# brucefan1983/GPUMD

Measured on AMD Instinct MI355X. Metric: atom-steps/sec, NEP PbTe NVE (nep4 2 Te Pb, examples/nep_train/nep.txt), higher is better.
Workload: dtype f32

## Files before the change

### gpumd_amd/csrc/capi_impl.h

```cpp
#pragma once
#include "../../include/nepmi.h"
#include "engine_impl.h"

#include <exception>
#include <string>

struct nepmi_api;
#if defined(NEPMI_CAPI_DISPATCH)
extern "C" const nepmi_api nepmi_self_api;
#define NEPMI_SELF_API (&nepmi_self_api)
#else
#define NEPMI_SELF_API nullptr
#endif

struct nepmi_model {
  const nepmi_api* api;
  nepmi::NepModel m;
};

struct nepmi_engine {
  const nepmi_api* api;
  nepmi::EngineT<NepmiBackend>* e;
};

// ... 981 lines not shown
  const std::string n(name);
  const int iv = (int)value;
  auto& eng = *e->e;
  if (n == "generic")
    return guarded([&] { eng.set_force_generic(iv != 0); });
  if (n == "tiles")
    eng.set_tile_mode(iv < 0 ? -1 : iv > 2 ? 2 : iv);
  else if (n == "win_lanes")
    eng.set_win_lanes(iv);
  else if (n == "win_max_atoms")
    eng.set_win_max_atoms(iv);
  else if (n == "scatter_guard")
    eng.set_scatter_guard_delayed(value, eng.take_guard_delay());
  else if (n == "scatter_guard_hard")
    eng.set_scatter_guard(-1.0, value);
  else if (n == "scatter_guard_delay")
    eng.set_guard_delay(iv);
  else if (n == "radial_mask")
    eng.set_radial_mask(iv != 0);
  else if (n == "radial_sync")
    eng.set_radial_sync(iv != 0);
  else if (n == "angular_fused")
    eng.set_angular_fused(iv != 0);
  else if (n == "angular_pair_trip")
    eng.set_angular_pair_trip(iv != 0);
  else if (n == "angular_flat_tables")
    eng.set_angular_flat_tables(iv != 0);
  else if (n == "lean_list_walks")
    eng.set_lean_list_walks(iv != 0);
  else if (n == "angular_only_list_a")
    eng.set_angular_only_list_a(iv != 0);
  else if (n == "rebuild_fast_pack")
    eng.set_rebuild_fast_pack(iv != 0);
  else if (n == "fold_seam")
    eng.set_fold_seam(iv != 0);
  else if (n == "brick_force") {
    if (iv != 0 && !eng.has_brick_force())
      return fail(NEPMI_ERR_ARG, "option 'brick_force': the per-brick force kernel is not part of this build (make BRICK=1)");
    eng.set_brick_force(iv != 0);
  }
  else if (n == "win_static")
    eng.set_win2(iv != 0);
  else if (n == "keep_lists_on_box_change")
    eng.set_keep_lists(iv != 0);
  else if (n == "stepwise_loops")
    eng.set_stepwise_loops(iv != 0);
  else if (n == "mfma")
    eng.set_use_mfma(iv);
  else if (n == "angular_recompute")
    eng.set_angular_recompute(iv);
  else
    return fail(NEPMI_ERR_ARG, "unknown engine option '" + n + "'");
  return NEPMI_OK;
}

}
```

### gpumd_amd/csrc/engine.hip

```cpp
#include <hip/hip_runtime.h>
#include <hiprand/hiprand_kernel.h>

#include <cstring>
#include <stdexcept>
#include <string>

#include "engine_impl.h"
#include "nep_scatter.h"
#include "nep_fused.h"
#ifndef NEPMI_WITH_BRICK
#define NEPMI_WITH_BRICK 0
#endif
#if NEPMI_WITH_BRICK
#include "experimental/nep_brick.h"
#endif

namespace nepmi {

#define NEPMI_HIP_CHECK(expr)                                                                       \
  do {                                                                                              \
    hipError_t err__ = (expr);                                                                      \
    if (err__ != hipSuccess)                                                                        \
      throw std::runtime_error(std::string("HIP error: ") + hipGetErrorString(err__) + " at " +     \
                               __FILE__ + ":" + std::to_string(__LINE__) + " (" #expr ")");         \
// ... 325 lines not shown
  body.lds_stage(nepmi_lds_pairs_s, tid, BLOCK);
  if (tid < 64)
    hist[tid] = 0;
  const unsigned per_xcd = gridDim.x >> 3;
  const unsigned tile = (blockIdx.x & 7u) * per_xcd + (blockIdx.x >> 3);
  const int64_t base = (int64_t)tile * (BLOCK / 2);
  const int j = tid >> 1;
  const bool live = base + j < n;
  int key = 0;
  if (live) {
    key = body.sort_key(base + j);
    key = key > 63 ? 63 : key;
    if (tile & 1u)
      key = 63 - key;
  }
  __syncthreads();
  if (live && (tid & 1) == 0)
    atomicAdd(&hist[key], 1);
  __syncthreads();
  if (tid == 0) {
    int run = 0;
    for (int c = 63; c >= 0; --c) {
      const int h = hist[c];
      hist[c] = run;
      run += h;
    }
  }
  __syncthreads();
  if (live && (tid & 1) == 0)
    perm[atomicAdd(&hist[key], 1)] = (unsigned short)j;
  __syncthreads();
  if (live)
    body.template run_parts<2>(base + perm[j], tid & 1, (lds_cfloat_ptr)nepmi_lds_pairs_s);
}

template <class Body>
__global__ void __launch_bounds__(256) nepmi_fused_image(const Body body, float* img)
{
  body.lds_stage(img, (int)threadIdx.x, 256);
}

template <int BLOCK, int P, class Body>
__global__ void __launch_bounds__(BLOCK) nepmi_kernel_lds_parts(const Body body, const int64_t n, const int* frozen)
{
  extern __shared__ __attribute__((aligned(16))) float nepmi_lds_parts[];
  if (frozen && *frozen != 0)
    return;
  const unsigned per_xcd = gridDim.x >> 3;
  const unsigned tile = (blockIdx.x & 7u) * per_xcd + (blockIdx.x >> 3);
  const int64_t i = ((int64_t)tile * BLOCK + threadIdx.x) / P;
  if (i < n)
    body.template run_parts<P>(i, (int)(threadIdx.x % P), (lds_cfloat_ptr)nepmi_lds_parts);
}

template <int BLOCK>
__device__ __forceinline__ int block_exclusive_scan(int v, int* total);

template <class Body>
__global__ void __launch_bounds__(kWinThreads) __attribute__((amdgpu_waves_per_eu(Body::kMinWavesPerEu)))
nepmi_win_kernel(const Body body, const int64_t nbricks)
{
  extern __shared__ __attribute__((aligned(16))) char nepmi_win_lds[];
  NEPMI_LDS(char)* lds = (NEPMI_LDS(char)*)nepmi_win_lds;
  if (body.skip())
    return;
  const unsigned per_xcd = gridDim.x >> 3;
// ... 1109 lines not shown
    const bool t = timed(slot);
    if (t)
      timer_start(timing->slot[slot]);
    hipLaunchKernelGGL((nepmi_kernel_lds_parts<BLOCK, P, Body>), dim3((unsigned)grid), dim3(BLOCK), lds_bytes, stream, body, n,
                       frozen);
    NEPMI_HIP_CHECK(hipGetLastError());
    if (t)
      timer_stop(timing->slot[slot]);
  }

  template <int BLOCK, class Body, bool SORTED = false>
  void launch_lds_pairs(int slot, int64_t n, const Body& body)
  {
    if (n <= 0)
      return;
    const int64_t grid = ((2 * n + BLOCK - 1) / BLOCK + 7) / 8 * 8;
    const size_t lds_bytes = ((size_t)body.lds_floats() * sizeof(float) + 15) / 16 * 16;
    void (*kern)(const Body, const int64_t, const int*) = nullptr;
    if constexpr (SORTED)
      kern = &nepmi_kernel_lds_pairs_sorted<BLOCK, Body>;
    else
      kern = &nepmi_kernel_lds_pairs<BLOCK, Body>;
    if (lds_bytes > 60 * 1024)
      NEPMI_HIP_CHECK(hipFuncSetAttribute(reinterpret_cast<const void*>(kern), hipFuncAttributeMaxDynamicSharedMemorySize, (int)lds_bytes));
    const bool t = timed(slot);
    if (t)
      timer_start(timing->slot[slot]);
    hipLaunchKernelGGL(kern, dim3((unsigned)grid), dim3(BLOCK), lds_bytes, stream, body, n, frozen);
    NEPMI_HIP_CHECK(hipGetLastError());
    if (t)
      timer_stop(timing->slot[slot]);
  }

  template <class S>
  size_t fused_image_floats(const ModelD& md, bool flat = false) const
  {
    return (size_t)fused_lds_layout<S>(md, 0, flat ? 1 : 0).total;
  }
  template <class S>
  void launch_angular_fused(int slot, int64_t n, const ModelD& md, const Bufs& b, int export_qfp, float* img, bool build, bool pair_trip,
                            bool flat = false)
  {
    if (build) {
      if (flat)
        hipLaunchKernelGGL((nepmi_fused_image<AngularFusedBody<S, 0, 1>>), dim3(1), dim3(256), 0, stream,
                           AngularFusedBody<S, 0, 1>{md, b, export_qfp, nullptr}, img);
      else
        hipLaunchKernelGGL((nepmi_fused_image<AngularFusedBody<S>>), dim3(1), dim3(256), 0, stream,
                           AngularFusedBody<S>{md, b, export_qfp, nullptr}, img);
      NEPMI_HIP_CHECK(hipGetLastError());
    }
#ifndef NEPMI_AFU_BLOCK
#define NEPMI_AFU_BLOCK 256
#endif
#ifndef NEPMI_AFU_SORT
#define NEPMI_AFU_SORT 0
#endif
    constexpr bool kTrips = FusedShape<S>::NLOC <= kFusedTripMaxChannels;
    if (flat) {
      if constexpr (kTrips) {
        if (pair_trip) {
          launch_lds_pairs<NEPMI_AFU_BLOCK, AngularFusedBody<S, 1, 1>, NEPMI_AFU_SORT != 0>(slot, n, AngularFusedBody<S, 1, 1>{md, b, export_qfp, img});
          return;
        }
      }
      launch_lds_pairs<NEPMI_AFU_BLOCK, AngularFusedBody<S, 0, 1>, NEPMI_AFU_SORT != 0>(slot, n, AngularFusedBody<S, 0, 1>{md, b, export_qfp, img});
      return;
    }
    if constexpr (kTrips) {
      if (pair_trip) {
        launch_lds_pairs<NEPMI_AFU_BLOCK, AngularFusedBody<S, 1>, NEPMI_AFU_SORT != 0>(slot, n, AngularFusedBody<S, 1>{md, b, export_qfp, img});
        return;
      }
    }
    launch_lds_pairs<NEPMI_AFU_BLOCK, AngularFusedBody<S>, NEPMI_AFU_SORT != 0>(slot, n, AngularFusedBody<S>{md, b, export_qfp, img});
  }

  template <class S>
  size_t fused_window_lds_bytes(const ModelD& md) const
  {
    return (size_t)fused_lds_layout<S>(md, kFusedWindowTypes).total * sizeof(float);
  }
  static constexpr bool kHasFusedWindow = NEPMI_WITH_FUSED_WINDOW != 0;
  template <class S>
  void launch_angular_fused_window(int slot, int64_t n, const ModelD& md, const Bufs& b, int export_qfp, float* img, bool build)
  {
#if NEPMI_WITH_FUSED_WINDOW
    if (n <= 0)
      return;
    AngularFusedBody<S> body{md, b, export_qfp, nullptr};
    if (build) {
      hipLaunchKernelGGL((nepmi_fused_image<AngularFusedBody<S>>), dim3(1), dim3(256), 0, stream, body, img);
      NEPMI_HIP_CHECK(hipGetLastError());
    }
    body.img = img;
    body.tw = kFusedWindowTypes;
    const int64_t grid = ((n + 127) / 128 + 7) / 8 * 8;
    const size_t lds_bytes = (fused_window_lds_bytes<S>(md) + 15) / 16 * 16;
    if (lds_bytes > 64 * 1024)
      NEPMI_HIP_CHECK(hipFuncSetAttribute(reinterpret_cast<const void*>(&nepmi_fused_window_kernel<AngularFusedBody<S>>),
                                          hipFuncAttributeMaxDynamicSharedMemorySize, (int)lds_bytes));
    const bool t = timed(slot);
    if (t)
      timer_start(timing->slot[slot]);
    hipLaunchKernelGGL((nepmi_fused_window_kernel<AngularFusedBody<S>>), dim3((unsigned)grid), dim3(256), lds_bytes, stream, body, n, frozen);
    NEPMI_HIP_CHECK(hipGetLastError());
    if (t)
      timer_stop(timing->slot[slot]);
// ... 428 lines not shown
```

### gpumd_amd/csrc/engine_impl.h

```cpp
#pragma once
#include "nep_bodies.h"
#include "nep_md.h"
#include "nep_corr.h"
#include "nep_rdf.h"
#include "nep_adf.h"
#include "nep_orient.h"
#include "nep_model.h"
#include "nep_window.h"
#include "nep_highl.h"
#include "tersoff_bodies.h"

#include <cmath>
#include <cstdio>
#include <cstring>
#include <string>
#include <random>
#include <vector>

#ifndef NEPMI_TERSOFF_SEAM
#define NEPMI_TERSOFF_SEAM 1
#endif
#ifndef NEPMI_WIN2_DEFAULT
#define NEPMI_WIN2_DEFAULT 1
#endif
// ... 1514 lines not shown
          const int64_t nc = set_grid();
          be_.memset(b_.cell_count, 0, sizeof(int) * (nc + 1));
          be_.memset(b_.flags + kFlagMaxBrick, 0, sizeof(int));
          be_.template launch<256>(kSlotMisc, N_, BinAtomsBody{box_, b_, pos});
          be_.template launch<64>(kSlotMisc, nc / 64, BrickMaxBody{b_});
          int fullest = 0;
          be_.sync();
          be_.d2h(&fullest, b_.flags + kFlagMaxBrick, sizeof(int));
          if (fullest <= kBrickFill)
            best = rc_cell;
        }
        grid_edge_ = best;
        grid_n_ = N_;
        for (int k = 0; k < 9; ++k)
          grid_h_[k] = box_.h[k];
      }
      rc_cell = grid_edge_;
      bin_grid();
      ncell = set_grid();
    }
    set_metric(false);
    be_.memset(b_.cell_count, 0, sizeof(int) * (ncell + 1));
    be_.memset(b_.cell_fill, 0, sizeof(int) * ncell);
    be_.memset(b_.cell_ghost, 0, sizeof(int) * ncell);
    const bool fast = rebuild_fast_pack_;
    static_assert(kFlagMaxAng == kFlagMaxSkin + 1 && kFlagMaxWindow == kFlagMaxAng + 1 && kFlagMaxCell == kFlagMaxWindow + 2, "adjacent flag words");
    if (fast) {
      be_.memset(b_.flags + kFlagMaxSkin, 0, 5 * sizeof(int));
    } else {
      be_.memset(b_.flags + kFlagMaxSkin, 0, 2 * sizeof(int));
    }
    be_.memset(b_.flags + kFlagMoved, 0, sizeof(int));
    be_.memset(b_.flags + kFlagOutlier, 0, sizeof(int));
    be_.begin_region(kRegionRebuild);
    be_.template launch<256>(kSlotMisc, N_, BinAtomsBody{box_, b_, pos});
    be_.exclusive_scan(b_.cell_count, ncell + 1, scan_scratch_);
    be_.template launch<256>(kSlotMisc, N_, FillCellsBody{b_});
    be_.template launch<256>(kSlotMisc, ncell, SortCellsBody{b_});
    be_.template launch<256>(kSlotMisc, N_, GatherSortedBody{box_, b_, pos, type});
    if (fuse_ann_active()) {
      be_.template launch<256>(kSlotMisc, N_, IdentityOrderBody{b_});
    } else {
      const int64_t nkeys = ((N_ >> kTypeChunkShift) + 1) * model_.num_types;
      be_.memset(b_.tcount, 0, sizeof(int) * (nkeys + 1));
      be_.template launch<64>(kSlotMisc, nkeys, TypeCountBody{b_, model_.num_types});
      be_.exclusive_scan(b_.tcount, nkeys + 1, scan_scratch_);
      be_.template launch<256>(kSlotMisc, N_, TypeFillBody{b_, model_.num_types});
    }
    if (!fast)
      be_.memset(b_.flags + kFlagMaxWindow, 0, 3 * sizeof(int));
    num_bricks_ = (int64_t)b_.gbx * b_.gby * b_.gbz;
    b_.brick_live = (b_.level && brick_live_buf_) ? brick_live_buf_ : nullptr;
    if (b_.level) {
      be_.memset(brick_live_buf_, 0, sizeof(int) * (size_t)(num_bricks_ + 1));
      be_.template launch<256>(kSlotMisc, N_, MarkGhostCellsBody{b_});
    }
    bool wave_stats = false;
    if constexpr (B::kHasScatter) {
      if (fast) {
        be_.launch_tile_stats_wave(kSlotMisc, num_bricks_, box_, b_);
        wave_stats = true;
      }
    }
    if (!wave_stats)
      be_.template launch<64>(kSlotMisc, num_bricks_, TileStatsBody{box_, b_});
    be_.memset(b_.brick_flag + num_bricks_, 0, sizeof(int));
// ... 166 lines not shown
  }
  bool ang_fused_window_active() const
  {
    if (!B::kHasFusedWindow || !B::kHasFusedAngular || !ang_fused_ || model_.kind != 0 || shape_ == 0 || ann_mode_ != 1 || model_.num_types <= 4 || !b_.fpr)
      return false;
    if ((model_.n_max_angular + 2) / 2 > 5)
      return false;
    const int nrh = (model_.n_max_radial + 2) / 2, nloc = (model_.n_max_angular + 2) / 2;
    const int dph = (nrh + model_.num_L * nloc + 3) / 4 * 4;
    const size_t T = (size_t)model_.num_types, tw = 4;
    const size_t floats = tw * ((size_t)model_.num_neurons * 2 * dph + 32 + 2 * model_.num_neurons) + 2 * dph +
                          tw * T * ((model_.n_max_angular + 1) * (model_.basis_size_angular + 1) + 1) + 16;
    return floats * sizeof(float) <= 80 * 1024;
  }
  template <class S>
  void launch_angular_fused_window(int export_qfp = 0)
  {
    if constexpr (B::kHasFusedWindow && B::kHasFusedAngular && S::fixed && S::TS == 0) {
      const size_t need = be_.template fused_image_floats<S>(md_);
      if (!fused_img_ || fused_img_floats_ < need) {
        dfree(fused_img_);
        fused_img_ = dalloc<float>(need);
        fused_img_floats_ = need;
        fused_img_stale_ = true;
      }
      be_.template launch_angular_fused_window<S>(kSlotAngular, N_, md_, b_, export_qfp, fused_img_, fused_img_stale_);
      fused_img_stale_ = false;
    }
  }
  template <class S>
  void launch_angular_fused(int export_qfp = 0, bool classic_image = false)
  {
    if constexpr (B::kHasFusedAngular && S::fixed) {
      if (ang_flat_tables_ && !classic_image) {
        const size_t need = be_.template fused_image_floats<S>(md_, true);
        if (!fused_img_flat_ || fused_img_flat_floats_ < need) {
          dfree(fused_img_flat_);
          fused_img_flat_ = dalloc<float>(need);
          fused_img_flat_floats_ = need;
          fused_img_flat_stale_ = true;
        }
        be_.template launch_angular_fused<S>(kSlotAngular, N_, md_, b_, export_qfp, fused_img_flat_, fused_img_flat_stale_, ang_pair_trip_, true);
        fused_img_flat_stale_ = false;
        last_ang_flat_ = true;
        return;
      }
      const size_t need = be_.template fused_image_floats<S>(md_);
      if (!fused_img_ || fused_img_floats_ < need) {
        dfree(fused_img_);
        fused_img_ = dalloc<float>(need);
        fused_img_floats_ = need;
        fused_img_stale_ = true;
      }
      be_.template launch_angular_fused<S>(kSlotAngular, N_, md_, b_, export_qfp, fused_img_, fused_img_stale_, ang_pair_trip_);
      fused_img_stale_ = false;
      last_ang_flat_ = false;
    }
  }

  template <class S>
  bool brick_force_wanted(const WinStage& ws2) const
  {
    if constexpr (!(B::kHasBrickForce && S::fixed && S::TS == 2)) {
      return false;
    } else {
      if (!brick_force_ || !ang_fused_active() || b_.level || b_.use_rmask || b_.use_csync || !scatter_wanted<S>(ws2))
        return false;
      return be_.template brick_lds_bytes<S>(md_, win_.wmax) <= B::kMaxLdsBytes;
    }
  }
  template <class S>
  void launch_brick_force(const WinStage& ws2, const int* frozen)
  {
    if constexpr (B::kHasBrickForce && S::fixed && S::TS == 2) {
      if (fused_img_stale_ || !fused_img_) {
        launch_angular_fused<S>(0, true);
      }
      be_.template launch_brick_force<S>(kSlotAngular, kSlotForce, num_bricks_, N_, ws2, md_, halo_, fmap_, fold_rows_, step_outputs_,
                                         fused_img_, frozen);
    }
  }

  template <class S>
  void launch_angular_force()
  {
    const bool big_table = (size_t)cang_floats(md_) * sizeof(float) > 16 * 1024;
#ifndef NEPMI_AF_PAIRS_BIG
// ... 196 lines not shown
    temperature_ = temperature;
    const float qT = (float)temperature * m.q_scaler_temp;
    b0_eff_.resize(m.b0.size());
    for (size_t k = 0; k < m.b0.size(); ++k)
      b0_eff_[k] = m.b0[k] - m.w0_temp[k] * qT;
    be_.h2d(const_cast<float*>(md_.b0), b0_eff_.data(), sizeof(float) * b0_eff_.size());
    be_.ann_prepare(md_, b_);
    fused_img_stale_ = fused_img_flat_stale_ = true;
  }
  double temperature() const { return temperature_; }
  bool temperature_model() const { return model_.temperature_model; }
  int recompute_s() const
  {
    return recompute_mode_ < 0 ? (model_.MN_angular <= 16 ? 1 : 0) : (recompute_mode_ ? 1 : 0);
  }
  void adopt_from(const EngineT& o)
  {
    use_tiles_ = o.use_tiles_;
    tile_mode_ = o.tile_mode_;
    recompute_mode_ = o.recompute_mode_;
    win_lanes_ = o.win_lanes_;
    win_max_atoms_ = o.win_max_atoms_;
    use_win2_ = o.use_win2_;
    external_skin_ = o.external_skin_;
    force_form_ = o.force_form_;
    use_rmask_ = o.use_rmask_;
    use_csync_ = o.use_csync_;
    ang_fused_ = o.ang_fused_;
    ang_pair_trip_ = o.ang_pair_trip_;
    ang_flat_tables_ = o.ang_flat_tables_;
    lean_walks_ = o.lean_walks_;
    aonly_list_a_ = o.aonly_list_a_;
    rebuild_fast_pack_ = o.rebuild_fast_pack_;
    fold_seam_ = o.fold_seam_;
    brick_force_ = o.brick_force_;
    loop_ctx_ = o.loop_ctx_;
    scatter_disabled_ = o.scatter_disabled_;
    b_.scatter_limit = o.b_.scatter_limit;
    b_.fold_guard = o.b_.fold_guard;
    b_.scatter_hard = o.b_.scatter_hard;
    b_.fold_hard = o.b_.fold_hard;
    hard_factor_ = o.hard_factor_;
    hard_asked_ = o.hard_asked_;
    guard_delay_ = o.guard_delay_;
    guard_delayed_ = o.guard_delayed_;
    if (reverse_ghosts_ != o.reverse_ghosts_)
      set_reverse_ghosts(o.reverse_ghosts_);
    unwrapped_ = o.unwrapped_;
    nhc_fresh_ = o.nhc_fresh_;
    bdp_rng_ = o.bdp_rng_;
    bdp_iset_ = o.bdp_iset_;
    bdp_gset_ = o.bdp_gset_;
    lan_seed_ = o.lan_seed_;
    num_compute = o.num_compute;
    num_rebuild = o.num_rebuild;
    num_discarded = o.num_discarded;
    num_range_handovers = o.num_range_handovers;
    be_.adopt_options(o.be_);
    if (ann_mode_ != o.ann_mode_)
      set_use_mfma(o.ann_mode_);
    if (force_generic_ != o.force_generic_)
      set_force_generic(o.force_generic_);
    if (o.temperature_ != temperature_)
      set_temperature(o.temperature_);
    have_list_ = false;
  }
// ... 347 lines not shown
    b_.fold_hard = on ? (int)((hard_factor_ > 2.0 ? hard_factor_ : 2.0) * b_.scatter_limit * 4194304.0) : 0;
  }
  bool scatter_enabled() const { return !scatter_disabled_; }
  void clear_range_hard()
  {
    int ov = 0;
    be_.d2h(&ov, b_.flags + kFlagOverflow, sizeof(int));
    if (ov & kOverflowRangeHard) {
      ov &= ~kOverflowRangeHard;
      be_.h2d(b_.flags + kFlagOverflow, &ov, sizeof(int));
    }
  }
  void disable_scatter()
  {
    if (!scatter_disabled_)
      ++num_range_handovers;
    scatter_disabled_ = true;
    be_.memset(b_.flags + kFlagRange, 0, sizeof(int));
  }
  bool last_scatter_form() const { return last_scatter_form_; }
  void set_angular_fused(bool on) { ang_fused_ = on; }
  void set_angular_pair_trip(bool on) { ang_pair_trip_ = on; }
  bool ang_pair_trip_active() const { return ang_pair_trip_ && (model_.n_max_angular + 2) / 2 <= 4; }
  void set_angular_flat_tables(bool on) { ang_flat_tables_ = on; }
  void set_lean_list_walks(bool on) { lean_walks_ = on; }
  void set_angular_only_list_a(bool on)
  {
    if (on != aonly_list_a_)
      have_list_ = false;
    aonly_list_a_ = on;
  }
  bool aonly_list_a_active() const { return aonly_list_a_ && shape_ts() == 2 && !use_rmask_; }
  void set_rebuild_fast_pack(bool on) { rebuild_fast_pack_ = on; }
  template <class S>
  bool lean_radial() const
  {
    return lean_walks_ && S::TS > 0;
  }
  bool lean_scatter() const { return lean_walks_ && shape_ts() > 0; }
  void set_fold_seam(bool on) { fold_seam_ = on; }
  void set_brick_force(bool on) { brick_force_ = on; }
  static constexpr bool has_brick_force() { return B::kHasBrickForce; }
  void set_loop_context(bool on) { loop_ctx_ = on; }
  void set_step_outputs(bool on) { step_outputs_ = on; }
  bool loop_context() const { return loop_ctx_; }
  void exact_virials()
  {
    if (!virial_local_ || model_.kind != 0 || last_small_)
      return;
    be_.frozen = nullptr;
    NEPMI_SHAPE_DISPATCH(exact_virials_shape, 1, ())
  }
  bool virial_local() const { return virial_local_; }

private:
  template <class S>
  void compact_lists_shape()
  {
    const bool padded_rows = b_.use_csync != 0;
    force_kernels_shape<S>(kPhaseRadialOnly, nullptr);
    if (padded_rows)
      angular_kernels<S>();
  }
  template <class S>
  void exact_virials_shape()
  {
// ... 60 lines not shown
    std::string s;
    if (model_.kind == 1)
      return "potential=tersoff1989 kernels=bond_order+force(fp64)";
    if (shape_ == 6) {
      char jb[96];
      std::snprintf(jb, sizeof jb, "shape=jit(%d,%d,%d,%d,%d;%s)", model_.n_max_radial, model_.basis_size_radial, model_.n_max_angular,
                    model_.basis_size_angular, model_.num_L, model_.num_types <= 2 ? std::to_string(model_.num_types).c_str() : "T");
      s += jb;
    } else {
      if (shape_ == 7 || shape_ == 8 || shape_ == 9) {
        s += shape_ == 7 ? "shape=cover(8,12,8,12,6;T)" : (shape_ == 8 ? "shape=cover(12,16,10,12,6;T)" : "shape=cover(8,12,8,12,6;2)");
        if (model_.embedded()) {
          char eb[128];
          std::snprintf(eb, sizeof eb, "<-zero_padded_model(%d,%d,%d,%d,%d)", model_.file_n_max_radial, model_.file_basis_size_radial,
                        model_.file_n_max_angular, model_.file_basis_size_angular, model_.file_num_L);
          s += eb;
        }
      } else {
        s += std::string("shape=") + shapes[shape_ >= 0 && shape_ <= 5 ? shape_ : 0];
      }
    }
    if (last_small_)
      return s + " path=small_box(all image pairs)";
    const int lanes = win_lanes();
    const bool win2 = win2_ok_ && lanes == 1;
    s += tile_ok_ ? (win2 ? " window=lds_static" : " window=lds_scanned") : " window=none(gather kernels)";
    s += " lanes_per_atom=" + std::to_string(tile_ok_ ? lanes : 1);
    if (last_brick_)
      s += " force=one_kernel_per_brick(descriptor+ann+partial_forces+lds_scatter_of_own_halves,lane_pairs)";
    else if (last_ang_fused_ && last_ang_window_)
      s += " angular=descriptor+ann+partial_forces_in_one_kernel(lane_pairs,sums_in_registers,type_sorted,window_of_4_types)";
    else if (last_ang_fused_)
      s += std::string(" angular=descriptor+ann+partial_forces_in_one_kernel(lane_pairs,sums_in_registers") +
           (ang_pair_trip_active() ? ",two_record_trips" : "") + (last_ang_flat_ ? ",flat_tables)" : ")");
    else if (fuse_ann_active())
      s += " ann=fused_with_angular_descriptor(packed_fp32,no_mfma)";
    else if (ann_mode_ != 0 && b_.ann_img && (model_.num_types <= 4 || b_.skip_atab))
      s += model_.num_types > 4 ? " ann=mfma_f32_32x32x2(one_type_per_workgroup)" : " ann=mfma_f32_32x32x2";
    else
      s += " ann=per_atom";
    if (!last_ang_fused_) {
      s += (shape_ != 0 && model_.n_max_angular + 1 >= 7) ? " angular_force=lane_pairs" : " angular_force=one_lane";
      s += recompute_s() ? " angular_sums=recomputed" : " angular_sums=stored";
    }
    s += (tile_ok_ && win2 && shape_ts() > 0 && lean_walks_) ? " list_walks=lean" : " list_walks=classic";
    s += (tile_ok_ && win2 && aonly_built_) ? " list_a=angular_only" : " list_a=classic";
    s += rebuild_fast_pack_ ? (b_.tbits ? " rebuild=fast_pack(types_from_the_builder)" : " rebuild=fast_pack") : " rebuild=classic";
    s += (last_scatter_form_ && last_mask_form_)   ? " radial_list=inside_bits_over_the_verlet_words"
         : (last_scatter_form_ && last_sync_form_) ? " radial_list=wave_synchronous_words"
                                                   : " radial_list=compacted";
    s += last_scatter_form_ ? (last_fold_seam_ ? " force_assembly=lds_scatter_of_own_halves(fixed_point)+fold_in_integrator_pass"
                                               : " force_assembly=lds_scatter_of_own_halves(fixed_point)+fold") :
         last_rows_form_ ? " force_assembly=table_rows_in_lds"
                         : (last_fpj_form_ ? " force_assembly=neighbour_half_from_fp_rows" : " force_assembly=table_rows_gathered");
    if (num_seam_vetoes_ > 0)
      s += " seam_vetoes=" + std::to_string(num_seam_vetoes_);
    if (tile_ok_)
      s += " bricks=" + std::to_string(num_bricks_) + " window_slots=" + std::to_string(win_.wmax);
    return s;
  }
  void force_kernels(int phase, const int* frozen = nullptr)
  {
    be_.frozen = frozen;
    force_kernels_dispatch(phase, frozen);
    be_.frozen = nullptr;
    step_outputs_ = true;
    assembly_part_ = 0;
// ... 20 lines not shown
        be_.template launch_lds<kTersoffBlock>(kSlotRadial, N_, TersoffPartialBody{box_, tp_, b_, tb_});
      if (tersoff_defer_)
        tersoff_deferred_ = true;
      else
        be_.template launch<64>(kSlotForce, N_, TersoffAssembleBody{b_, tb_});
      be_.end_region(kRegionForce);
      return;
    }
    NEPMI_SHAPE_DISPATCH(force_kernels_shape, 1, (phase, frozen))
  }

  NepModel model_;
  B be_;
  int64_t cap_;
  int64_t N_;
  ModelD md_{};
  Bufs b_;
  BoxD box_;
  WinLayout win_{0, 0};
  bool win2_ok_ = false, use_win2_ = NEPMI_WIN2_DEFAULT != 0;
  bool use_rows_ = true;
  bool last_rows_form_ = false, last_fpj_form_ = false, last_scatter_form_ = false;
  int force_form_ = -1;
  bool loop_ctx_ = false;
  bool virial_local_ = false;
  double hard_factor_ = 4.0;
  bool ang_fused_ = true;
  bool ang_pair_trip_ = !(std::getenv("NEPMI_ANGULAR_PAIR_TRIP") && std::atoi(std::getenv("NEPMI_ANGULAR_PAIR_TRIP")) == 0);
  bool ang_flat_tables_ = !(std::getenv("NEPMI_ANGULAR_FLAT_TABLES") && std::atoi(std::getenv("NEPMI_ANGULAR_FLAT_TABLES")) == 0);
  bool lean_walks_ = !(std::getenv("NEPMI_LEAN_LIST_WALKS") && std::atoi(std::getenv("NEPMI_LEAN_LIST_WALKS")) == 0);
  bool aonly_list_a_ = !(std::getenv("NEPMI_ANGULAR_ONLY_LIST_A") && std::atoi(std::getenv("NEPMI_ANGULAR_ONLY_LIST_A")) == 0);
  bool aonly_built_ = false;
  bool rebuild_fast_pack_ = !(std::getenv("NEPMI_REBUILD_FAST_PACK") && std::atoi(std::getenv("NEPMI_REBUILD_FAST_PACK")) == 0);
  float* fused_img_flat_ = nullptr;
  size_t fused_img_flat_floats_ = 0;
  bool fused_img_flat_stale_ = true;
  bool last_ang_flat_ = false;
  bool brick_force_ = false;
  bool last_brick_ = false;
  bool brick_pending_ = false;
  float* fused_img_ = nullptr;
  size_t fused_img_floats_ = 0;
  bool fused_img_stale_ = true;
  bool last_ang_fused_ = false;
  bool use_rmask_ = false;
  bool last_mask_form_ = false;
  bool last_ang_window_ = false;
  bool last_sync_form_ = false;
  int guard_delay_ = 0;
  int guard_delay_next_ = 0;
  bool fold_seam_ = !(std::getenv("NEPMI_FOLD_SEAM") && std::atoi(std::getenv("NEPMI_FOLD_SEAM")) == 0);
  bool fold_defer_ = false;
  bool fold_deferred_ = false;
  static constexpr int kSeamBackoffSteps = 256;
  int seam_backoff_ = 0;
  int64_t num_seam_vetoes_ = 0;
  bool last_fold_seam_ = false;
  bool tersoff_defer_ = false;
  bool tersoff_deferred_ = false;
  int64_t calm_steps_ = 0;
  int* brick_live_buf_ = nullptr;
  double* thermo_rows_ = nullptr;
  int64_t thermo_rows_cap_ = 0;
  bool rev_valid_ = false;
  const int* dmap_dev_ = nullptr;
  double hard_asked_ = 4.0;
// ... 77 lines not shown
```

### gpumd_amd/csrc/nep_bodies.h

```cpp
#pragma once
#include <type_traits>

#include "nep_dev.h"

namespace nepmi {

struct alignas(16) F4 {
  float x, y, z;
  int w;
};

struct alignas(16) U4 {
  unsigned x, y, z, w;
};

struct alignas(16) WinRec {
  int x, y, z;
  int w;
};

struct WinGeom {
  double inv_unit;
  double cell_frac[3];
  int cv[9];
// ... 9 lines not shown
#define NEPMI_ATOMIC_MAX(ptr, v) atomicMax((ptr), (v))
#else
NEPMI_HD int host_fetch_add(int* p, int v) { int o = *p; *p = o + v; return o; }
#define NEPMI_ATOMIC_ADD(ptr, v) host_fetch_add((ptr), (v))
#define NEPMI_ATOMIC_OR(ptr, v) (*(ptr) |= (v))
#define NEPMI_ATOMIC_MAX(ptr, v) (*(ptr) = (*(ptr) > (v) ? *(ptr) : (v)))
#endif

template <int NR_, int KR_, int NA_, int KA_, int NL_, int TS_>
struct Shape {
  static constexpr int NR = NR_, KR = KR_, NA = NA_, KA = KA_, NL = NL_, TS = TS_;
  static constexpr bool fixed = NR_ >= 0;
  static constexpr int NRM = NR_ >= 0 ? NR_ : 19;
  static constexpr int KRM = KR_ >= 0 ? KR_ : 19;
  static constexpr int NAM = NA_ >= 0 ? NA_ : 19;
  static constexpr int KAM = KA_ >= 0 ? KA_ : 19;
  static constexpr int NLM = NL_ >= 0 ? NL_ : 14;
  static constexpr int kRows = NR_ >= 0 ? 6 : 14;
  static constexpr int DIMM = (NRM + 1) + (NAM + 1) * NLM;
};
using ShapeGeneric = Shape<-1, -1, -1, -1, -1, 0>;

enum FlagSlot {
  kFlagMoved = 0, kFlagOverflow = 1,
  kFlagRange = 2,
  kFlagMaxSkin = 3, kFlagMaxAng = 4,
  kFlagMaxWindow = 5, kFlagMaxBrick = 6, kFlagMaxCell = 7, kFlagNumBoundary = 8,
  kFlagOutlier = 9,
  kFlagFoldRows = 10,
  kFlagSeamVeto = 11,
  kNumFlags = 12
};
constexpr int kOverflowRangeHard = 16;

constexpr int kAngRowPad = 8;
constexpr int kNullRecord = -1;
struct Bufs {
  int64_t N;
  int nbx, nby, nbz;
  int gbx, gby, gbz;
  double rc_inv_cell;
  float rc_skin_sq;
  float rc_askin_sq;
  int* cell_count;
  int* cell_fill;
  int* cell_ghost;
  int* brick_live;
  int* brick_flag;
  int* brick_order;
  int* cid;
  int* perm;
  PosQ* posq;
  double* x0s;
  int MN_skin, MN_ang, MN_acomp;
  int MN_arows;
  int* nn_ang;   int* nl_ang;  unsigned short* rev_ang;
  int* nn_skin;  int* nl_skin;
  unsigned short* code_ang;
  unsigned short* code_skin;
  int* nn_rad;   F4* rstash;
  int* nn_angstep; F4* acomp;
  int* nn_angtrue;
  unsigned short* amap;
  F4* f12;
  float* q;
  float* fp;
// ... 2730 lines not shown
```

### gpumd_amd/nep.py

```python
import ctypes as C
import weakref

import numpy as np

from . import _capi


def _h9(box):
    h = np.ascontiguousarray(np.asarray(box, dtype=np.float64).reshape(9))
    return h, h.ctypes.data_as(_capi.c_dp)


def _pbc3(pbc):
    p = np.ascontiguousarray(np.asarray(pbc, dtype=np.int32).reshape(3))
    return p, p.ctypes.data_as(_capi.c_ip)


class Model:

    def __init__(self, path, lib=None):
        from . import load_library
        self.lib = lib if lib is not None else load_library()
        self.path = path
        self.handle = self.lib.nepmi_model_load(path.encode())
# ... 313 lines not shown
    def set_radial_mask(self, on=True):
        self.set_option("radial_mask", 1 if on else 0)

    def set_radial_sync(self, on=True):
        self.set_option("radial_sync", 1 if on else 0)

    def set_scatter_guard(self, ev_per_angstrom=64.0, hard_factor=0.0):
        self.set_option("scatter_guard", float(ev_per_angstrom))
        self.set_option("scatter_guard_hard", float(hard_factor))

    def set_virial_mode(self, mode=0):
        self._ck(self.lib.nepmi_engine_set_virial_mode(self.handle, int(mode)))

    def set_brick_force(self, on=True):
        self.set_option("brick_force", 1 if on else 0)

    def set_angular_fused(self, on=True):
        self.set_option("angular_fused", 1 if on else 0)

    def set_angular_pair_trip(self, on=True):
        self.set_option("angular_pair_trip", 1 if on else 0)

    def set_angular_flat_tables(self, on=True):
        self.set_option("angular_flat_tables", 1 if on else 0)

    def set_lean_list_walks(self, on=True):
        self.set_option("lean_list_walks", 1 if on else 0)

    def set_angular_only_list_a(self, on=True):
        self.set_option("angular_only_list_a", 1 if on else 0)

    def set_rebuild_fast_pack(self, on=True):
        self.set_option("rebuild_fast_pack", 1 if on else 0)

    def set_fold_seam(self, on=True):
        self.set_option("fold_seam", 1 if on else 0)

    def describe(self):
        import ctypes as C
        buf = C.create_string_buffer(1024)
        n = self.lib.nepmi_engine_describe(self.handle, buf, 1024)
        if n < 0:
            self._ck(n)
        return buf.value.decode()

    def set_stepwise_loops(self, on=True):
        self.set_option("stepwise_loops", int(bool(on)))

    def set_win_static(self, on=True):
        self.set_option("win_static", int(bool(on)))

    def set_mfma(self, on=True):
        self.set_option("mfma", int(on))

    def set_temperature(self, temperature):
        self._ck(self.lib.nepmi_engine_set_temperature(self.handle, float(temperature)))

    def set_angular_recompute(self, mode=-1):
        self.set_option("angular_recompute", int(mode))

    def set_generic(self, on=True):
        self.set_option("generic", 1 if on else 0)


def dos_from_mvac(lib, sums, group_size, dt_ps, omega_max, num_dos_points=None):
    sums = np.ascontiguousarray(sums, dtype=np.float64)
# ... 265 lines not shown
```

Measured before the change: 1.003 billion.

## Add persistent work-stealing launch for fused angular kernel with per-wave type sort

Adds a persistent-grid variant of the fused angular pair kernel. Each workgroup stages the LDS table image once, then its wavefronts pull units of work from eight atomic counters until they run dry. Inside each 64-atom group the atoms are sorted by key with ballots and lane permutes, so the lanes of a wave handle similar atom types. The point is to pay the LDS staging once per resident block rather than once per tile and to balance load dynamically. In exchange it adds atomic traffic, the cost of the in-wave sort, and a counter-reset protocol that depends on the last finishing wave.

```diff
diff --git a/gpumd_amd/csrc/capi_impl.h b/gpumd_amd/csrc/capi_impl.h
--- a/gpumd_amd/csrc/capi_impl.h
+++ b/gpumd_amd/csrc/capi_impl.h
@@ -1037,6 +1037,8 @@
     eng.set_angular_only_list_a(iv != 0);
   else if (n == "rebuild_fast_pack")
     eng.set_rebuild_fast_pack(iv != 0);
+  else if (n == "angular_persistent")
+    eng.set_angular_persistent(iv);
   else if (n == "fold_seam")
     eng.set_fold_seam(iv != 0);
   else if (n == "brick_force") {
diff --git a/gpumd_amd/csrc/engine.hip b/gpumd_amd/csrc/engine.hip
--- a/gpumd_amd/csrc/engine.hip
+++ b/gpumd_amd/csrc/engine.hip
@@ -381,6 +381,111 @@
   __syncthreads();
   if (live)
     body.template run_parts<2>(base + perm[j], tid & 1, (lds_cfloat_ptr)nepmi_lds_pairs_s);
+}
+
+#ifndef NEPMI_AFU_GROUP
+#define NEPMI_AFU_GROUP 64
+#endif
+constexpr int kAfuGroup = NEPMI_AFU_GROUP;
+constexpr int kAfuCounters = 8;
+template <int BLOCK, class Body>
+__global__ void __launch_bounds__(BLOCK) __attribute__((amdgpu_waves_per_eu(Body::kMinWavesPerEuPairs)))
+nepmi_kernel_lds_pairs_persistent(const Body body, const int64_t n, const int* frozen, unsigned* ctr, const unsigned nunits)
+{
+  static_assert(BLOCK % 64 == 0, "whole wavefronts");
+  static_assert(kAfuGroup == 0 || kAfuGroup == 64 || kAfuGroup == 128, "keys per lane: one or two");
+  extern __shared__ __attribute__((aligned(16))) float nepmi_lds_pairs_p[];
+  if (frozen && *frozen != 0)
+    return;
+  body.lds_stage(nepmi_lds_pairs_p, (int)threadIdx.x, BLOCK);
+  __syncthreads();
+  const int lane = (int)(threadIdx.x & 63u);
+  const unsigned per = (nunits + kAfuCounters - 1) / kAfuCounters;
+  for (unsigned rr = 0; rr < (unsigned)kAfuCounters; ++rr) {
+    const unsigned r = (blockIdx.x + rr) & (unsigned)(kAfuCounters - 1);
+    const unsigned lo = r * per;
+    if (lo >= nunits)
+      continue;
+    const unsigned cnt = nunits - lo < per ? nunits - lo : per;
+    for (;;) {
+      unsigned t = 0;
+      if (lane == 0)
+        t = atomicAdd(&ctr[r], 1u);
+      t = (unsigned)__builtin_amdgcn_readfirstlane((int)t);
+      if (t >= cnt)
+        break;
+      const unsigned u = lo + t;
+      int64_t k;
+      if constexpr (kAfuGroup == 0) {
+        k = (int64_t)u * 32 + (lane >> 1);
+      } else {
+        constexpr int K = kAfuGroup ? kAfuGroup / 64 : 1, PARTS = 2 * K;
+        const int64_t base = (int64_t)(u / PARTS) * (64 * K);
+        const int part = (int)(u % PARTS);
+        int key[K], rank[K];
+        unsigned long long rem[K];
+#pragma unroll
+        for (int j = 0; j < K; ++j) {
+          const int64_t a = base + 64 * j + lane;
+          key[j] = a < n ? body.sort_key(a) : -1;
+          rank[j] = 0;
+          rem[j] = ~0ull;
+        }
+        for (;;) {
+          int v;
+          if (rem[0] != 0ull) {
+            v = __builtin_amdgcn_readlane(key[0], __builtin_ctzll(rem[0]));
+          } else {
+            if constexpr (K == 2) {
+              if (rem[1] == 0ull)
+                break;
+              v = __builtin_amdgcn_readlane(key[1], __builtin_ctzll(rem[1]));
+            } else {
+              break;
+            }
+          }
+          int front = 0, total = 0;
+          unsigned long long m[K];
+#pragma unroll
+          for (int j = 0; j < K; ++j) {
+            m[j] = __ballot(key[j] == v);
+            rem[j] &= ~m[j];
+            total += __popcll(m[j]);
+          }
+#pragma unroll
+          for (int j = 0; j < K; ++j) {
+            const int before = (int)__builtin_amdgcn_mbcnt_hi((unsigned)(m[j] >> 32), __builtin_amdgcn_mbcnt_lo((unsigned)m[j], 0u));
+            rank[j] += key[j] < v ? total : (key[j] == v ? front + before : 0);
+            front += __popcll(m[j]);
+          }
+        }
+        int got = 0;
+#pragma unroll
+        for (int j = 0; j < K; ++j) {
+          const int dst = (rank[j] >> 5) == part ? (rank[j] & 31) : 32 + (lane & 31);
+          got |= __builtin_amdgcn_ds_permute(dst << 2, 64 * j + lane + 1);
+        }
+        got = __builtin_amdgcn_ds_bpermute((lane >> 1) << 2, got);
+        k = (unsigned)(got - 1) < (unsigned)(64 * K) ? base + (got - 1) : n;
+      }
+      if (k < n) {
+        using KBody = const __attribute__((address_space(4))) Body;
+        KBody* kp = (KBody*)__builtin_amdgcn_kernarg_segment_ptr();
+        asm volatile("" : "+s"(kp));
+        int part = lane & 1;
+        asm volatile("" : "+v"(part));
+        ((const Body*)kp)->template run_parts<2>(k, part, (lds_cfloat_ptr)nepmi_lds_pairs_p);
+      }
+    }
+  }
+  unsigned fin = 0;
+  if (lane == 0)
+    fin = atomicAdd(&ctr[kAfuCounters], 1u);
+  if (lane == 0 && fin + 1u == gridDim.x * (unsigned)(BLOCK / 64)) {
+#pragma unroll
+    for (int c = 0; c <= kAfuCounters; ++c)
+      atomicExch(&ctr[c], 0u);
+  }
 }
 
 template <class Body>
@@ -1556,6 +1661,64 @@
       timer_stop(timing->slot[slot]);
   }
 
+#ifndef NEPMI_AFU_BLOCK
+#define NEPMI_AFU_BLOCK 256
+#endif
+#ifndef NEPMI_AFU_SORT
+#define NEPMI_AFU_SORT 0
+#endif
+  static_assert(nepmi::kAfuCtrWords == kAfuCounters + 1, "the engine's counter buffer: a word per range and the done word");
+  template <int BLOCK, class Body>
+  void launch_lds_pairs_persistent(int slot, int64_t n, const Body& body, int workgroups, unsigned* ctr)
+  {
+    if (n <= 0)
+      return;
+    constexpr int64_t kGroup = kAfuGroup ? kAfuGroup : 32;
+    const int64_t nunits = (n + kGroup - 1) / kGroup * (kGroup / 32);
+    if (nunits > 0x7fffffff)
+      throw EngineError{-4, "fused angular kernel: too many atoms for the unit counters"};
+    const size_t lds_bytes = ((size_t)body.lds_floats() * sizeof(float) + 15) / 16 * 16;
+    auto kern = &nepmi_kernel_lds_pairs_persistent<BLOCK, Body>;
+    static thread_local size_t asked_lds = ~(size_t)0;
+    static thread_local int64_t resident = 0;
+    if (asked_lds != lds_bytes) {
+      if (lds_bytes > 60 * 1024)
+        NEPMI_HIP_CHECK(hipFuncSetAttribute(reinterpret_cast<const void*>(kern), hipFuncAttributeMaxDynamicSharedMemorySize, (int)lds_bytes));
+      int dev = 0, cus = 0, per_cu = 0;
+      NEPMI_HIP_CHECK(hipGetDevice(&dev));
+      NEPMI_HIP_CHECK(hipDeviceGetAttribute(&cus, hipDeviceAttributeMultiprocessorCount, dev));
+      NEPMI_HIP_CHECK(hipOccupancyMaxActiveBlocksPerMultiprocessor(&per_cu, reinterpret_cast<const void*>(kern), BLOCK, lds_bytes));
+      resident = (int64_t)(per_cu > 0 ? per_cu : 1) * (cus > 0 ? cus : 1);
+      asked_lds = lds_bytes;
+    }
+    int64_t grid = workgroups < 0 ? -(int64_t)workgroups : workgroups > 1 ? workgroups : resident;
+    const int64_t most = (nunits + BLOCK / 64 - 1) / (BLOCK / 64);
+    grid = grid < most ? grid : most;
+    const bool t = timed(slot);
+    if (t)
+      timer_start(timing->slot[slot]);
+    hipLaunchKernelGGL(kern, dim3((unsigned)grid), dim3(BLOCK), lds_bytes, stream, body, n, frozen, ctr, (unsigned)nunits);
+    NEPMI_HIP_CHECK(hipGetLastError());
+    if (t)
+      timer_stop(timing->slot[slot]);
+  }
+  template <class S>
+  static constexpr bool afu_persistent_shape()
+  {
+    return FusedShape<S>::NLOC <= kFusedTripMaxChannels;
+  }
+  template <class Body>
+  void launch_afu_shell(int slot, int64_t n, const Body& body, int persistent, unsigned* ctr)
+  {
+    if constexpr (Body::kRoomy) {
+      if (persistent != 0 && ctr) {
+        launch_lds_pairs_persistent<NEPMI_AFU_BLOCK, Body>(slot, n, body, persistent, ctr);
+        return;
+      }
+    }
+    launch_lds_pairs<NEPMI_AFU_BLOCK, Body, NEPMI_AFU_SORT != 0>(slot, n, body);
+  }
+
   template <class S>
   size_t fused_image_floats(const ModelD& md, bool flat = false) const
   {
@@ -1563,7 +1726,7 @@
   }
   template <class S>
   void launch_angular_fused(int slot, int64_t n, const ModelD& md, const Bufs& b, int export_qfp, float* img, bool build, bool pair_trip,
-                            bool flat = false)
+                            bool flat = false, int persistent = 0, unsigned* ctr = nullptr)
   {
     if (build) {
       if (flat)
@@ -1574,30 +1737,24 @@
                            AngularFusedBody<S>{md, b, export_qfp, nullptr}, img);
       NEPMI_HIP_CHECK(hipGetLastError());
     }
-#ifndef NEPMI_AFU_BLOCK
-#define NEPMI_AFU_BLOCK 256
-#endif
-#ifndef NEPMI_AFU_SORT
-#define NEPMI_AFU_SORT 0
-#endif
     constexpr bool kTrips = FusedShape<S>::NLOC <= kFusedTripMaxChannels;
     if (flat) {
       if constexpr (kTrips) {
         if (pair_trip) {
-          launch_lds_pairs<NEPMI_AFU_BLOCK, AngularFusedBody<S, 1, 1>, NEPMI_AFU_SORT != 0>(slot, n, AngularFusedBody<S, 1, 1>{md, b, export_qfp, img});
+          launch_afu_shell(slot, n, AngularFusedBody<S, 1, 1>{md, b, export_qfp, img}, persistent, ctr);
           return;
         }
       }
-      launch_lds_pairs<NEPMI_AFU_BLOCK, AngularFusedBody<S, 0, 1>, NEPMI_AFU_SORT != 0>(slot, n, AngularFusedBody<S, 0, 1>{md, b, export_qfp, img});
+      launch_afu_shell(slot, n, AngularFusedBody<S, 0, 1>{md, b, export_qfp, img}, persistent, ctr);
       return;
     }
     if constexpr (kTrips) {
       if (pair_trip) {
-        launch_lds_pairs<NEPMI_AFU_BLOCK, AngularFusedBody<S, 1>, NEPMI_AFU_SORT != 0>(slot, n, AngularFusedBody<S, 1>{md, b, export_qfp, img});
+        launch_afu_shell(slot, n, AngularFusedBody<S, 1>{md, b, export_qfp, img}, persistent, ctr);
         return;
       }
     }
-    launch_lds_pairs<NEPMI_AFU_BLOCK, AngularFusedBody<S>, NEPMI_AFU_SORT != 0>(slot, n, AngularFusedBody<S>{md, b, export_qfp, img});
+    launch_afu_shell(slot, n, AngularFusedBody<S>{md, b, export_qfp, img}, persistent, ctr);
   }
 
   template <class S>
diff --git a/gpumd_amd/csrc/engine_impl.h b/gpumd_amd/csrc/engine_impl.h
--- a/gpumd_amd/csrc/engine_impl.h
+++ b/gpumd_amd/csrc/engine_impl.h
@@ -1570,6 +1570,8 @@
     }
     be_.memset(b_.flags + kFlagMoved, 0, sizeof(int));
     be_.memset(b_.flags + kFlagOutlier, 0, sizeof(int));
+    if (afu_ctr_)
+      be_.memset(afu_ctr_, 0, sizeof(unsigned) * kAfuCtrWords);
     be_.begin_region(kRegionRebuild);
     be_.template launch<256>(kSlotMisc, N_, BinAtomsBody{box_, b_, pos});
     be_.exclusive_scan(b_.cell_count, ncell + 1, scan_scratch_);
@@ -1802,6 +1804,12 @@
   void launch_angular_fused(int export_qfp = 0, bool classic_image = false)
   {
     if constexpr (B::kHasFusedAngular && S::fixed) {
+      constexpr bool kPersistentShape = B::template afu_persistent_shape<S>();
+      if (kPersistentShape && ang_persistent_ != 0 && !afu_ctr_) {
+        afu_ctr_ = dalloc<unsigned>(kAfuCtrWords);
+        be_.memset(afu_ctr_, 0, sizeof(unsigned) * kAfuCtrWords);
+      }
+      last_ang_persistent_ = kPersistentShape && ang_persistent_ != 0;
       if (ang_flat_tables_ && !classic_image) {
         const size_t need = be_.template fused_image_floats<S>(md_, true);
         if (!fused_img_flat_ || fused_img_flat_floats_ < need) {
@@ -1810,7 +1818,8 @@
           fused_img_flat_floats_ = need;
           fused_img_flat_stale_ = true;
         }
-        be_.template launch_angular_fused<S>(kSlotAngular, N_, md_, b_, export_qfp, fused_img_flat_, fused_img_flat_stale_, ang_pair_trip_, true);
+        be_.template launch_angular_fused<S>(kSlotAngular, N_, md_, b_, export_qfp, fused_img_flat_, fused_img_flat_stale_, ang_pair_trip_, true,
+                                             ang_persistent_, afu_ctr_);
         fused_img_flat_stale_ = false;
         last_ang_flat_ = true;
         return;
@@ -1822,7 +1831,8 @@
         fused_img_floats_ = need;
         fused_img_stale_ = true;
       }
-      be_.template launch_angular_fused<S>(kSlotAngular, N_, md_, b_, export_qfp, fused_img_, fused_img_stale_, ang_pair_trip_);
+      be_.template launch_angular_fused<S>(kSlotAngular, N_, md_, b_, export_qfp, fused_img_, fused_img_stale_, ang_pair_trip_, false,
+                                           ang_persistent_, afu_ctr_);
       fused_img_stale_ = false;
       last_ang_flat_ = false;
     }
@@ -2085,6 +2095,7 @@
     lean_walks_ = o.lean_walks_;
     aonly_list_a_ = o.aonly_list_a_;
     rebuild_fast_pack_ = o.rebuild_fast_pack_;
+    ang_persistent_ = o.ang_persistent_;
     fold_seam_ = o.fold_seam_;
     brick_force_ = o.brick_force_;
     loop_ctx_ = o.loop_ctx_;
@@ -2498,6 +2509,7 @@
   }
   bool aonly_list_a_active() const { return aonly_list_a_ && shape_ts() == 2 && !use_rmask_; }
   void set_rebuild_fast_pack(bool on) { rebuild_fast_pack_ = on; }
+  void set_angular_persistent(int v) { ang_persistent_ = v; }
   template <class S>
   bool lean_radial() const
   {
@@ -2624,7 +2636,8 @@
       s += " angular=descriptor+ann+partial_forces_in_one_kernel(lane_pairs,sums_in_registers,type_sorted,window_of_4_types)";
     else if (last_ang_fused_)
       s += std::string(" angular=descriptor+ann+partial_forces_in_one_kernel(lane_pairs,sums_in_registers") +
-           (ang_pair_trip_active() ? ",two_record_trips" : "") + (last_ang_flat_ ? ",flat_tables)" : ")");
+           (ang_pair_trip_active() ? ",two_record_trips" : "") + (last_ang_flat_ ? ",flat_tables)" : ")") +
+           (last_ang_persistent_ ? " angular_shell=persistent" : " angular_shell=tiles");
     else if (fuse_ann_active())
       s += " ann=fused_with_angular_descriptor(packed_fp32,no_mfma)";
     else if (ann_mode_ != 0 && b_.ann_img && (model_.num_types <= 4 || b_.skip_atab))
@@ -2711,6 +2724,9 @@
   bool aonly_list_a_ = !(std::getenv("NEPMI_ANGULAR_ONLY_LIST_A") && std::atoi(std::getenv("NEPMI_ANGULAR_ONLY_LIST_A")) == 0);
   bool aonly_built_ = false;
   bool rebuild_fast_pack_ = !(std::getenv("NEPMI_REBUILD_FAST_PACK") && std::atoi(std::getenv("NEPMI_REBUILD_FAST_PACK")) == 0);
+  int ang_persistent_ = std::getenv("NEPMI_ANGULAR_PERSISTENT") ? std::atoi(std::getenv("NEPMI_ANGULAR_PERSISTENT")) : 1;
+  unsigned* afu_ctr_ = nullptr;
+  bool last_ang_persistent_ = false;
   float* fused_img_flat_ = nullptr;
   size_t fused_img_flat_floats_ = 0;
   bool fused_img_flat_stale_ = true;
diff --git a/gpumd_amd/csrc/nep_bodies.h b/gpumd_amd/csrc/nep_bodies.h
--- a/gpumd_amd/csrc/nep_bodies.h
+++ b/gpumd_amd/csrc/nep_bodies.h
@@ -65,6 +65,7 @@
   kNumFlags = 12
 };
 constexpr int kOverflowRangeHard = 16;
+constexpr int kAfuCtrWords = 9;
 
 constexpr int kAngRowPad = 8;
 constexpr int kNullRecord = -1;
diff --git a/gpumd_amd/nep.py b/gpumd_amd/nep.py
--- a/gpumd_amd/nep.py
+++ b/gpumd_amd/nep.py
@@ -369,6 +369,9 @@
 
     def set_rebuild_fast_pack(self, on=True):
         self.set_option("rebuild_fast_pack", 1 if on else 0)
+
+    def set_angular_persistent(self, value=1):
+        self.set_option("angular_persistent", int(value))
 
     def set_fold_seam(self, on=True):
         self.set_option("fold_seam", 1 if on else 0)
```

New measurement: 799.1 million. 0.796x the previous value.
